# kan-bayashi/espnet

Hardware: AMD Instinct MI355X
Metric: frames/sec, 12L Conformer hybrid CTC/attention training step (B=32 T=1000 d=256 per GPU) (higher is better)
Workload: dtype f32; 1 GPU; BASELINE configs[1]: 12L Conformer enc d=256 h=4 ff=2048 k=31 macaron+cnn rel_pos, 6L Transformer dec, V=5000, fbank B=32 T=1000 L=100, mtlalpha 0.3, lsm 0.1; global_batch=32, frames=1000, parallelism=dp1, optimizer=adam+noam, clip 5.0, launch=hipGraph, wgrad_side_stream=False, optimizer_steps_done=113

## Files before the change

### espnet_amd/csrc/gemm.hip

```cpp
#include <stdlib.h>
#include "common.h"
#include "../../include/espnet_amd.h"

namespace {

constexpr int BK = 32;
constexpr int NTHREADS = 256;

template <int BM, int BN, int PREC>
struct Smem {
  static constexpr int LDK = PREC ? 40 : 36;
  using elem_t = typename std::conditional<PREC == 1, unsigned short, float>::type;
  elem_t a[2][BM][LDK];
  elem_t b[2][BN][LDK];
  int poff[3][BK];
};

struct RowState {
  int base;
  int ih, jw;
  int ok;
};

__device__ __forceinline__ RowState decompose(const eamd_gather_t& g, int row, int nrows) {
// ... 295 lines not shown
          else if (p.epilogue == 3) v = p.aux[coff + prow * p.ldaux + n] > 0.f ? v : 0.f;
          else if (p.epilogue == 4) v *= eamd_dswish(p.aux[coff + prow * p.ldaux + n]);
          else if (p.epilogue == 5) v *= p.aux[coff + prow * p.ldaux + n];
          v *= p.alpha;
          if (p.R) v += p.R[coff + prow * p.ldr + n];
          float* cp = p.C + coff + prow * p.ldc + n;
          if (p.beta != 0.f) v += p.beta * (*cp);
          *cp = v;
        }
      }
    }
  }
}

template <int BM, int BN, int PREC>
int launch(const eamd_gemm_t& p, hipStream_t stream) {
  dim3 grid((p.M + BM - 1) / BM, (p.N + BN - 1) / BN, p.batch1 * p.batch2 * p.splitk);
  size_t smem = sizeof(Smem<BM, BN, PREC>);
  if (smem > 64 * 1024) {
    static const hipError_t attr_err = hipFuncSetAttribute(
        reinterpret_cast<const void*>(&gemm_kernel<BM, BN, PREC>), hipFuncAttributeMaxDynamicSharedMemorySize,
        (int)sizeof(Smem<BM, BN, PREC>));
    if (attr_err != hipSuccess) return (int)attr_err;
  }
  hipLaunchKernelGGL((gemm_kernel<BM, BN, PREC>), grid, dim3(NTHREADS), smem, stream, p);
  EAMD_LAUNCH_CHECK();
  return EAMD_OK;
}

}

int eamd_gemm_bf16_dispatch(const eamd_gemm_t& p, int tile, hipStream_t stream);
int eamd_gemm_f32_dispatch(const eamd_gemm_t& p, int tile, hipStream_t stream);

static int gemm_check(eamd_gemm_t& p, int& tile_out, const bool no_c = false) {
  const bool stats = p.epilogue == 7;
  const bool no_result = stats || no_c;
  const bool rowgrad = p.epilogue == 8;
  if (!p.A || !p.B || (!p.C && !p.Cb && !no_result)) return EAMD_EINVAL;
  if (stats && (!p.stats.part || !p.stats.zfix || (p.stats.col && !p.stats.zcol))) return EAMD_EINVAL;
  if (rowgrad && !p.stats.rowc) return EAMD_EINVAL;
  if ((stats || rowgrad) && (p.stats.fix < 0 || p.stats.fix >= p.N || (p.tile != 64 && p.tile != 128) || p.splitk > 1 ||
                             p.batch1 * p.batch2 != 1 || p.cmap.enabled || p.gather.enabled || p.Hb || p.drop_p != 0.f ||
                             p.R || p.colsum || p.beta != 0.f))
    return EAMD_EINVAL;
  if (p.in_dtype != 0 && p.in_dtype != 1) return EAMD_EINVAL;
  if (p.in_dtype == 1 && p.precision != 1) return EAMD_EINVAL;
  if (p.in_dtype == 0 && (p.Cb || p.aux_dtype || (!p.C && !no_result))) return EAMD_EUNSUPPORTED;
  if (p.M <= 0 || p.N <= 0 || p.K < 0) return EAMD_EINVAL;
  if (p.batch1 <= 0 || p.batch2 <= 0) return EAMD_EINVAL;
  if (p.splitk < 1) p.splitk = 1;
  if (p.splitk > 1 && p.epilogue != 0) return EAMD_EINVAL;
  if (p.epilogue < 0 || p.epilogue > 8) return EAMD_EINVAL;
  if (p.epilogue >= 3 && p.epilogue <= 5 && !p.aux) return EAMD_EINVAL;
  if (p.epilogue == 6 && (!p.Hb || p.drop_p <= 0.f)) return EAMD_EINVAL;
  if (p.precision != 0 && p.precision != 1) return EAMD_EINVAL;
  if ((long)p.batch1 * p.batch2 * p.splitk > 65535) return EAMD_EUNSUPPORTED;

  int tile = p.tile;
  if (tile == 0) {
    long t128 = (long)((p.M + 127) / 128) * ((p.N + 127) / 128) * p.batch1 * p.batch2 * p.splitk;
    if (p.in_dtype == 1) {
      constexpr int T128_KMIN = 320, T128_NMIN = 256;
      tile = (t128 >= 1024 && p.K >= T128_KMIN && p.M >= 2048 && p.N >= T128_NMIN) ? 128 : 64;
    } else {
      tile = (t128 >= (p.precision == 0 ? 240 : 512) && p.M >= 128 && p.N >= 128) ? 128 : 64;
      if (p.precision == 0 && tile == 128 && t128 > 256 && t128 < 400 && p.splitk == 1) tile = 64;
    }
  }
  if (tile != 64 && tile != 128) return EAMD_EINVAL;

  if (p.gather.enabled) {
    const eamd_gather_t& g = p.gather;
    if (g.ntap < 1 || g.ntap > 9 || g.C <= 0 || g.C % BK != 0) return EAMD_EINVAL;
    if (!p.transA) {
      if (p.K != g.ntap * g.C) return EAMD_EINVAL;
    } else {
      if (p.M != g.ntap * g.C) return EAMD_EINVAL;
      if (g.C % tile != 0) return EAMD_EINVAL;
    }
  }
  if (p.colsum && p.gather.enabled &&
      (!p.transA || !p.transB || p.in_dtype != 0 || p.batch1 * p.batch2 != 1 || p.a_act != EAMD_ACT_NONE || p.b_act != EAMD_ACT_NONE))
    return EAMD_EUNSUPPORTED;
  if ((p.N + tile - 1) / tile > 65535) return EAMD_EUNSUPPORTED;
  if (p.h_dtype != 0 && p.h_dtype != 1) return EAMD_EINVAL;
  if (p.in_dtype == 1 && p.h_dtype != 0) return EAMD_EUNSUPPORTED;
  if (p.in_dtype != 1 && ((p.Hb && !(p.h_dtype == 1 && p.precision == 0)) || (p.drop_p != 0.f && p.precision != 0)))
    return EAMD_EUNSUPPORTED;
  if ((p.a_act > EAMD_ACT_SWISH || p.b_act > EAMD_ACT_SWISH) && (p.in_dtype != 0 || p.precision != 0)) return EAMD_EUNSUPPORTED;
  tile_out = tile;
  return EAMD_OK;
}

extern "C" int eamd_gemm(const eamd_gemm_t* pp, void* stream_) {
  if (!pp) return EAMD_EINVAL;
  eamd_gemm_t p = *pp;
  hipStream_t stream = (hipStream_t)stream_;
  int tile = 0;
  const int chk = gemm_check(p, tile);
  if (chk != EAMD_OK) return chk;
  const bool stats = p.epilogue == 7, rowgrad = p.epilogue == 8;
  if (p.in_dtype == 1) return eamd_gemm_bf16_dispatch(p, tile, stream);

  if (p.precision == 1 && p.gather.enabled && p.transA && !p.Hb && p.drop_p == 0.f) {
    const int rc = eamd_gemm_f32_dispatch(p, tile, stream);
    if (rc != EAMD_EUNSUPPORTED) return rc;
  }
  if (p.precision == 0) {
    const int rc = eamd_gemm_f32_dispatch(p, tile, stream);
    if (rc != EAMD_EUNSUPPORTED) return rc;
    if (p.drop_p != 0.f || p.Hb || p.a_act > EAMD_ACT_SWISH || p.b_act > EAMD_ACT_SWISH) return EAMD_EUNSUPPORTED;
  }
  if (stats || rowgrad) return EAMD_EUNSUPPORTED;
  if (p.colsum && p.gather.enabled) return EAMD_EUNSUPPORTED;
  if (tile == 128) {
    return p.precision ? launch<128, 128, 1>(p, stream) : launch<128, 128, 0>(p, stream);
  }
  return p.precision ? launch<64, 64, 1>(p, stream) : launch<64, 64, 0>(p, stream);
}

int eamd_gemm_f32_multi(const eamd_gemm_t* ps, const int* tiles, int n, hipStream_t stream);

extern "C" int eamd_gemm_multi(const eamd_gemm_t* descs, int n, void* stream) {
  if (!descs || n < 1) return EAMD_EINVAL;
  if (n >= 2 && n <= EAMD_GEMM_MULTI_MAX) {
    eamd_gemm_t ps[EAMD_GEMM_MULTI_MAX];
    int tiles[EAMD_GEMM_MULTI_MAX];
    bool f32 = true;
    for (int i = 0; i < n; ++i) {
      ps[i] = descs[i];
      const int chk = gemm_check(ps[i], tiles[i]);
      if (chk != EAMD_OK) return chk;
      f32 = f32 && ps[i].in_dtype == 0 && ps[i].precision == 0;
    }
    if (f32) {
      const int rc = eamd_gemm_f32_multi(ps, tiles, n, (hipStream_t)stream);
      if (rc != EAMD_EUNSUPPORTED) return rc;
    }
  }
  for (int i = 0; i < n; ++i) {
    const int rc = eamd_gemm(&descs[i], stream);
    if (rc != EAMD_OK) return rc;
  }
  return EAMD_OK;
}

int eamd_gemm_f32_conv1w(const eamd_gemm_t* ps, const int* tiles, int n, const float* x, int T, int F, float* part, int* nslab,
                         hipStream_t stream);
int eamd_conv1_bwd_w_reduce(const float* part, int nslab, int C, float* dw, float* db, hipStream_t stream);

extern "C" int eamd_conv2_bwd_x_conv1_bwd_w(const eamd_gemm_t* descs, int n, const float* x, int T, int F, float* part,
// ... 47 lines not shown
```

### espnet_amd/csrc/gemm_f32.hip

```cpp
#include <stdlib.h>
#include <type_traits>
#include "common.h"
#include "../../include/espnet_amd.h"

#include "gemm_bf16_common.h"

namespace {

constexpr int FBK = 32;

template <int BM, int BN, bool TA, bool TB>
struct SmemF {
  static constexpr int KPAD_A = BM >= 128 ? 8 : 4, KPAD_B = BN >= 128 ? 8 : 4;
  static constexpr int LDA = TA ? BM + KPAD_A : FBK + 4;
  static constexpr int RA = TA ? FBK : BM;
  static constexpr int LDB = TB ? BN + KPAD_B : FBK + 4;
  static constexpr int RB = TB ? FBK : BN;
  static constexpr int OPS = 2 * (RA * LDA + RB * LDB);
  static constexpr int CT = BM * (BN + 4);
  float ab[OPS > CT ? OPS : CT];
  int poff[8][FBK];
  __device__ float* a(int buf) { return ab + buf * RA * LDA; }
  __device__ float* b(int buf) { return ab + 2 * RA * LDA + buf * RB * LDB; }
};
// ... 673 lines not shown
}

template <int T>
int dispatch_layout_f(const eamd_gemm_t& p, hipStream_t s) {
  if (p.transA) return p.transB ? launch_f<T, T, true, true, false>(p, s) : launch_f<T, T, true, false, false>(p, s);
  return p.transB ? launch_f<T, T, false, true, false>(p, s) : launch_f<T, T, false, false, false>(p, s);
}

bool aligned16f(const void* q) { return (reinterpret_cast<uintptr_t>(q) & 15) == 0; }

}

int eamd_gemm_f32_dispatch(const eamd_gemm_t& p, int tile, hipStream_t stream) {
  if (p.Cb || (p.Hb && !p.h_dtype) || p.aux_dtype || (!p.C && p.epilogue != 7)) return EAMD_EUNSUPPORTED;
  if (p.Hb && p.drop_p <= 0.f) return EAMD_EINVAL;
  if (p.drop_p < 0.f || p.drop_p >= 1.f) return EAMD_EINVAL;
  if (p.drop_p > 0.f && (p.cmap.enabled || p.batch1 * p.batch2 != 1 || p.ldc != p.N || p.splitk > 1)) return EAMD_EINVAL;
  const bool a_ok = aligned16f(p.A) && p.lda % 4 == 0 && p.sA1 % 4 == 0 && p.sA2 % 4 == 0 &&
                    p.lda >= (p.transA ? (p.M + 3) / 4 * 4 : (p.K + 3) / 4 * 4);
  const bool b_ok = aligned16f(p.B) && p.ldb % 4 == 0 && p.sB1 % 4 == 0 && p.sB2 % 4 == 0 &&
                    p.ldb >= (p.transB ? (p.N + 3) / 4 * 4 : (p.K + 3) / 4 * 4);
  if (p.gather.enabled) {
    const eamd_gather_t& g = p.gather;
    if (g.C % FBK != 0 || !p.transB || !aligned16f(p.A) || !b_ok) return EAMD_EUNSUPPORTED;
    if (p.a_act != EAMD_ACT_NONE || p.b_act != EAMD_ACT_NONE) return EAMD_EUNSUPPORTED;
    if (!gather_taps_small(g)) return EAMD_EUNSUPPORTED;
    if (p.transA && g.C % tile != 0) return EAMD_EUNSUPPORTED;
    if (tile == 128)
      return p.transA ? launch_f<128, 128, true, true, true>(p, stream) : launch_f<128, 128, false, true, true>(p, stream);
    return p.transA ? launch_f<64, 64, true, true, true>(p, stream) : launch_f<64, 64, false, true, true>(p, stream);
  }
  if (!a_ok || !b_ok) return EAMD_EUNSUPPORTED;
  return tile == 128 ? dispatch_layout_f<128>(p, stream) : dispatch_layout_f<64>(p, stream);
}

template <bool NOPAD>
static int multi_launch_t(const MultiF& m, int grid, hipStream_t stream) {
  constexpr size_t smem = sizeof(SmemF<128, 128, false, true>);
  static const hipError_t attr_err = hipFuncSetAttribute(
      reinterpret_cast<const void*>(&gemm_f32_multi_kernel<128, 128, false, true, true, NOPAD>),
      hipFuncAttributeMaxDynamicSharedMemorySize, (int)smem);
  if (attr_err != hipSuccess) return (int)attr_err;
  hipLaunchKernelGGL((gemm_f32_multi_kernel<128, 128, false, true, true, NOPAD>), dim3((unsigned)grid), dim3(NT_), smem, stream, m);
  EAMD_LAUNCH_CHECK();
  return EAMD_OK;
}

int eamd_gemm_f32_multi(const eamd_gemm_t* ps, const int* tiles, int n, hipStream_t stream) {
  if (n < 2 || n > EAMD_GEMM_MULTI_MAX) return EAMD_EUNSUPPORTED;
  MultiF m;
  bool nopad = true;
  int maxnt = 0;
  for (int i = 0; i < n; ++i) {
    const eamd_gemm_t& p = ps[i];
    if (tiles[i] != 128 || p.in_dtype != 0 || p.precision != 0) return EAMD_EUNSUPPORTED;
    if (!p.gather.enabled || p.transA || !p.transB || p.splitk != 1 || p.batch1 * p.batch2 != 1) return EAMD_EUNSUPPORTED;
    if (!p.C || p.Cb || p.Hb || p.aux_dtype || p.epilogue > 5 || p.colsum) return EAMD_EUNSUPPORTED;
    if (p.a_act != EAMD_ACT_NONE || p.b_act != EAMD_ACT_NONE || p.drop_p != 0.f) return EAMD_EUNSUPPORTED;
    const bool b_ok = aligned16f(p.B) && p.ldb % 4 == 0 && p.ldb >= (p.N + 3) / 4 * 4;
    if (p.gather.C % FBK != 0 || !aligned16f(p.A) || !b_ok || !gather_taps_small(p.gather)) return EAMD_EUNSUPPORTED;
    const long nt = (long)((p.M + 127) / 128) * ((p.N + 127) / 128);
    if (nt > (1L << 24)) return EAMD_EUNSUPPORTED;
    nopad = nopad && gather_nopad(p.gather);
    m.p[i] = p;
    m.nt[i] = (int)nt;
    maxnt = nt > maxnt ? (int)nt : maxnt;
// ... 95 lines not shown
```

### espnet_amd/functional.py

```python
import math

import torch

from . import ops
from .ops import (ACT_NONE, ACT_RELU, ACT_SWISH, EPI_DACT_FACTOR, EPI_MUL_AUX, EPI_MUL_DSWISH, EPI_MUL_RELU_MASK, EPI_NONE,
                  EPI_RELU)


class GradSink:

    on_done = None
    on_use = None

    @staticmethod
    def use(params):
        if GradSink.on_use is not None and torch.is_grad_enabled():
            GradSink.on_use(params)
        return params

    def __init__(self, params):
        self.params = list(params)
        self.ret = [None] * len(self.params)

    def buf(self, i):
# ... 584 lines not shown
        adt = ops.act_dtype()
        inp2 = ops.to_act_shared(inp).reshape(-1, Din)
        W = ops.wshadow(ws[0]).detach().as_strided((rows_w, Din), (Din, 1))
        b = bs[0].detach().as_strided((rows_w,), (1,)) if bs else None
        out = ops.linear_fwd(inp2, W, b, out_dtype=adt)
        sp = SharedProj(out, nblk, zero_grad, torch.float32 if zero_grad else adt)
        box.append(sp)
        ctx.sp, ctx.inp2, ctx.W, ctx.shape = sp, inp2, W, inp.shape
        ctx.pr = GradSink.use(params)
        ctx.n_w = n_w
        return torch.zeros((), device=inp.device)

    @staticmethod
    def backward(ctx, _dtoken):
        sp, inp2, W = ctx.sp, ctx.inp2, ctx.W
        params = ctx.pr
        ws, bs = params[:ctx.n_w], params[ctx.n_w:]
        blocks = sorted(sp.pending)
        sp.pending = []
        dinp = None
        if blocks:
            assert blocks == list(range(blocks[0], blocks[-1] + 1)), "consumers of one backward pass are consecutive blocks"
            lo, hi = blocks[0] * sp.width, (blocks[-1] + 1) * sp.width
            M, Din, n = inp2.shape[0], inp2.shape[1], hi - lo
            dy = sp.dout if sp.dout.dtype == inp2.dtype else ops.to_act(sp.dout)
            rows_w = W.shape[0]
            dW = ws[0]._eamd_grad.as_strided((rows_w, Din), (Din, 1))[lo:hi]
            db = bs[0]._eamd_grad.as_strided((rows_w,), (1,))[lo:hi] if bs else None
            sk = ops.auto_splitk(n, Din, M)
            ops.gemm(dy, inp2, dW, n, Din, M, sp.ld, Din, Din, transA=1, transB=1, splitk=sk,
                     beta=1.0 if sk == 1 else 0.0, colsum=db, a_off=lo)
            if ctx.needs_input_grad[0]:
                dinp = torch.empty(M, Din, device=inp2.device, dtype=torch.float32)
                ops.gemm(dy, W, dinp, M, Din, n, sp.ld, Din, Din, transB=1, a_off=lo, b_off=lo * Din)
                dinp = dinp.view(ctx.shape)
            sp.done += len(blocks)
        if sp.done >= sp.n and GradSink.on_done is not None:
            ops.wgrad_join()
            GradSink.on_done(params)
        return (dinp, None, None, None, None) + (None,) * len(params)


class MHABlockFn(torch.autograd.Function):

    @staticmethod
    def forward(ctx, x, memory, pos_emb, mask, H, eps, last_query_only, drop, pre, token, *params):
        p_att, s_att, p_out, s_out = drop
        pre_kv = pre if (pre is not None and pre[0] == "kv") else None
        pre_pos = pre if (pre is not None and pre[0] == "pos") else None
        ln_w, ln_b, wq, bq, wk, bk, wv, bv, wo, bo = params[:10]
        rel = len(params) > 10
        B, T1f, D = x.shape
        dk = D // H
        adt = ops.act_dtype()
        x2 = x.reshape(-1, D).contiguous()
        fused = memory is None and not last_query_only and _qkv_adjacent(wq, wk, wv, bq, bk, bv)
        rp = None
        if fused and eps is not None and D == 256 and x2.dtype == torch.float32 and adt == torch.float32 \
                and ops.rowproj_ok(x2.shape[0], D, 3 * D) and (p_out <= 0.0 or ops.f32_epilogue_drop()):
            w3 = _span3(ops.wshadow(wq), (3 * D, D))
            rp = ops.rowproj_images(wq, [(w3, False), (w3, True), (wo.detach(), False), (wo.detach(), True)])
        if rp is not None:
            xn = torch.empty_like(x2)
            mean = torch.empty(x2.shape[0], device=x2.device, dtype=torch.float32)
            rstd = torch.empty_like(mean)
        else:
            xn, mean, rstd = _ln_fwd_in(x2, ln_w, ln_b, eps, adt)
# ... 638 lines not shown
```

### espnet_amd/ops.py

```python
import ctypes as C
import os
import math

import torch

from . import _lib
from ._lib import GatherT, GemmT, RowMapT, check, ptr, stream_ptr

ACT_NONE, ACT_RELU, ACT_SWISH = 0, 1, 2
EPI_NONE, EPI_RELU, EPI_SWISH, EPI_MUL_RELU_MASK, EPI_MUL_DSWISH, EPI_MUL_AUX, EPI_DACT_FACTOR, EPI_ROW_STATS, EPI_ROW_GRAD = 0, 1, 2, 3, 4, 5, 6, 7, 8

_PRECISIONS = {"fp32": 0, "bf16": 1}
_state = {"precision": 0}


def set_precision(name):
    if name not in _PRECISIONS:
        raise ValueError(f"precision must be one of {list(_PRECISIONS)}")
    _state["precision"] = _PRECISIONS[name]


def get_precision():
    return [k for k, v in _PRECISIONS.items() if v == _state["precision"]][0]

# ... 49 lines not shown


def _span(rows, ld, cols):
    return (rows - 1) * ld + cols if rows > 0 else 0


_time_bound = {"t": None}


def set_time_bound(t):
    if t is not None and not (t.is_cuda and t.dtype == torch.int32 and t.numel() == 1):
        raise _lib.EamdError("time bound: one int32 element on the device")
    _time_bound["t"] = t


def time_bound():
    return _time_bound["t"]


def mask_time(x, T, bound):
    rows = x.numel() // x.shape[-1]
    assert x.is_contiguous() and rows % T == 0 and x.dtype in (torch.float32, torch.bfloat16)
    check(_lib.lib().eamd_mask_time(ptr(x), rows, x.shape[-1], T, ptr(bound), x.dtype == torch.bfloat16,
                                    stream_ptr()), "eamd_mask_time")
    return x


_gemm_record = None


def gemm(A, B, Cm, M, N, K, lda, ldb, ldc, *, transA=0, transB=0, bias=None, aux=None, ldaux=0, R=None,
         ldr=0, batch=(1, 1), sA=(0, 0), sB=(0, 0), sC=(0, 0), alpha=1.0, beta=0.0, a_act=0, b_act=0,
         epilogue=0, splitk=1, tile=0, gather=None, cmap=None, a_off=0, b_off=0, c_off=0, precision=None,
         colsum=None, Cb=None, drop=None, Hb=None, h_act=0, group=False, stats=None, defer=None):
    bf = A.dtype == torch.bfloat16
    if A.dtype != B.dtype or A.dtype not in (torch.float32, torch.bfloat16) or not (A.is_cuda and B.is_cuda):
        raise _lib.EamdError("gemm needs float32 or bfloat16 GPU operands of one dtype")
    if stats is not None:
        assert epilogue in (EPI_ROW_STATS, EPI_ROW_GRAD) and tile in (64, 128) and splitk == 1
        assert (Cm is None and Cb is None) if epilogue == EPI_ROW_STATS else Cm is not None
    c32 = Cm if (Cm is not None and Cm.dtype == torch.float32) else None
    c16 = Cb if Cb is not None else (Cm if (Cm is not None and Cm.dtype == torch.bfloat16) else None)
    if c16 is not None and (c16.dtype != torch.bfloat16 or not bf):
        raise _lib.EamdError("gemm: bf16 outputs need bf16 operands")
    for tt in (R, bias, colsum):
        if tt is not None and tt.dtype != torch.float32:
            raise _lib.EamdError("gemm: bias / residual / colsum must be float32")
    b1, b2 = batch
    if gather is None:
        a_span = _span(K, lda, M) if transA else _span(M, lda, K)
        a_need = a_off + (b1 - 1) * sA[0] + (b2 - 1) * sA[1] + a_span
        if a_need > A.numel():
            raise _lib.EamdError(f"gemm: A too small ({A.numel()} < {a_need})")
    b_span = _span(K, ldb, N) if transB else _span(N, ldb, K)
    b_need = b_off + (b1 - 1) * sB[0] + (b2 - 1) * sB[1] + b_span
    if b_need > B.numel():
        raise _lib.EamdError(f"gemm: B too small ({B.numel()} < {b_need})")
    if cmap is None:
        c_need = c_off + (b1 - 1) * sC[0] + (b2 - 1) * sC[1] + _span(M, ldc, N)
        for ct in (c32, c16):
            if ct is not None and c_need > ct.numel():
                raise _lib.EamdError(f"gemm: C too small ({ct.numel()} < {c_need})")
    if bias is not None and bias.numel() < N:
        raise _lib.EamdError("gemm: bias too small")

    p = GemmT()
    p.A, p.B = ptr(A, a_off), ptr(B, b_off)
# ... 9 lines not shown
                raise _lib.EamdError("gemm: colsum with a gather needs transA, transB, float32 operands and N outputs")
        elif not transA or colsum.numel() < M * b1 * b2:
            raise _lib.EamdError("gemm: colsum needs transA and M outputs")
        p.colsum = ptr(colsum)
    p.M, p.N, p.K = M, N, K
    p.transA, p.transB = int(transA), int(transB)
    p.lda, p.ldb, p.ldc, p.ldaux, p.ldr = lda, ldb, ldc, ldaux or ldc, ldr or ldc
    p.batch1, p.batch2 = b1, b2
    p.sA1, p.sA2 = sA
    p.sB1, p.sB2 = sB
    p.sC1, p.sC2 = sC
    p.alpha, p.beta = alpha, beta
    p.a_act, p.b_act, p.epilogue = a_act, b_act, epilogue
    p.splitk = splitk
    p.in_dtype = 1 if bf else 0
    p.precision = 1 if bf else (_state["precision"] if precision is None else precision)
    p.tile = tile
    if stats is not None and epilogue == EPI_ROW_GRAD:
        rowc, col, fix, gscale, scale = stats
        if rowc.dtype != torch.float32 or rowc.numel() < 3 * M or col.dtype != torch.int32 or col.numel() < M or not (0 <= fix < N):
            raise _lib.EamdError("gemm: row-gradient coefficients too small or of the wrong dtype")
        p.stats.rowc, p.stats.col, p.stats.fix, p.stats.gscale, p.stats.scale = ptr(rowc), ptr(col), int(fix), ptr(gscale), float(scale)
    elif stats is not None:
        part, col, zcol, zfix, fix = stats
        tn = (N + tile - 1) // tile
        if part.dtype != torch.float32 or part.numel() < M * tn * 2 or zfix.numel() < M or not (0 <= fix < N) or \
                (col is not None and (col.dtype != torch.int32 or col.numel() < M or zcol is None or zcol.numel() < M)):
            raise _lib.EamdError("gemm: row-statistics buffers too small or of the wrong dtype")
        p.stats.part, p.stats.col, p.stats.zcol, p.stats.zfix, p.stats.fix = ptr(part), ptr(col), ptr(zcol), ptr(zfix), int(fix)
    if gather is not None:
        p.gather = gather
    if cmap is not None:
        p.cmap = cmap
    if drop is not None and drop[0] > 0.0:
        if ldc != N or c_off != 0 or (not bf and p.precision != 0):
            raise _lib.EamdError("gemm: fused dropout needs a contiguous [M, N] result and bf16 or fp32-MFMA operands")
        p.drop_p, p.drop_salt = float(drop[0]), int(drop[1])
        p.drop_step = ptr(rng_state(A.device))
        if Hb is not None:
            if Hb.dtype != (torch.bfloat16 if bf else torch.float32) or Hb.numel() < M * N:
                raise _lib.EamdError("gemm: Hb must be an [M, N] buffer of the operand dtype")
            p.Hb, p.h_act, p.h_dtype = ptr(Hb), h_act, 0 if bf else 1
    if group and _wgroup["on"] and _in_grad_arena(Cm) and _wgroup_accepts(p):
        lo = Cm.data_ptr() + 4 * c_off
        hi = lo + 4 * _span(M, ldc, N)
        nbytes = A.numel() * A.element_size() + B.numel() * B.element_size()
        clash = any(lo < qhi and qlo < hi and (splitk == 1 or qsk == 1) for qlo, qhi, qsk in _wgroup["ranges"])
        if clash or _wgroup["bytes"] + nbytes > GROUP_WGRAD_MAX_BYTES:
            wgrad_group_flush()
        _wgroup["items"].append((p, (A, B, Cm, colsum)))
        _wgroup["ranges"].append((lo, hi, splitk))
        _wgroup["bytes"] += nbytes
        return
    if defer is not None:
        defer.append((p, (A, B, Cm, bias, aux, R, colsum, Cb, Hb, stats)))
        return
    if _gemm_record is not None:
        _gemm_record.append((p, (A, B, Cm, bias, aux, R, colsum, Cb, Hb, stats),
                             lambda sp, p=p: check(_lib.lib().eamd_gemm(C.byref(p), sp), "eamd_gemm")))
    check(_lib.lib().eamd_gemm(C.byref(p), stream_ptr()), "eamd_gemm")


GEMM_MULTI_MAX = 4


def gemm_multi(items):
# ... 187 lines not shown
        with inference():
            return fn(*a, **k)
    return wrapped
LINEAR_ROWS_MAX = 16
LINEAR_ROWS_BLOCK_MAX = 1024
LINEAR_ROWS_KSPLIT = True


def linear_fwd(x, W, b, out=None, *, act=EPI_NONE, R=None, alpha=1.0, a_act=ACT_NONE, out_dtype=torch.float32,
               drop=None, Hb=None, h_act=ACT_NONE):
    M, K = x.shape
    N = W.shape[0]
    assert W.shape[1] == K and W.is_contiguous() and x.stride(1) == 1 and (R is None or R.stride(-1) == 1)
    if (LINEAR_ROWS and (M <= LINEAR_ROWS_MAX or (M <= LINEAR_ROWS_BLOCK_MAX and (K <= 512 or (K >= 1024 and LINEAR_ROWS_KSPLIT)) and N <= 1024
                                                  and K % 16 == 0)) and out is None and out_dtype == torch.float32 and x.dtype == torch.float32 and W.dtype == torch.float32
            and act in (EPI_NONE, EPI_RELU, EPI_SWISH) and a_act in (ACT_NONE, ACT_RELU, ACT_SWISH) and drop is None and Hb is None
            and K % 4 == 0 and _state["precision"] == 0 and _infer > 0 and not torch.is_grad_enabled()
            and (R is None or (tuple(R.shape) == (M, N) and (M == 1 or R.stride(0) >= N))) and (M == 1 or x.stride(0) >= K)):
        y = torch.empty(M, N, device=x.device, dtype=torch.float32)
        rc = _lib.lib().eamd_linear_rows_f32(ptr(x), ptr(W), ptr(b), ptr(R), ptr(y), M, N, K, a_act, act, alpha,
                                             x.stride(0), R.stride(0) if R is not None else 0, stream_ptr())
        if rc == 0:
            return y
        if rc != _lib.EAMD_EUNSUPPORTED:
            check(rc, "eamd_linear_rows_f32")
    x = x.contiguous()
    R = R.contiguous() if R is not None else None
    sk = 1
    if (out_dtype if out is None else out.dtype) == torch.float32 and act == EPI_NONE and drop is None and Hb is None:
        if R is None and alpha == 1.0:
            sk = _skinny_splitk(M, N, K)
        elif K >= 1024 and M <= 512 and x.is_cuda and torch.cuda.is_current_stream_capturing():
            sk = _skinny_splitk(M, N, K, max_rows=512)
    if out is None:
        out = zeros(M, N, device=x.device) if sk > 1 else torch.empty(M, N, device=x.device, dtype=out_dtype)
    elif sk > 1:
        out.zero_()
    gemm(x, W, out, M, N, K, K, K, N, bias=b, epilogue=act, R=R, ldr=N, alpha=alpha, a_act=a_act, drop=drop, Hb=Hb,
         h_act=h_act, splitk=sk)
    return out


class _ZeroArena:
    buf = None
    off = 0
    need = 0
    cap = 0
    active = False
    tracking = False
    capture = 0


_zarena = _ZeroArena()
ZERO_ARENA = True
ZERO_ARENA_MAX = 1024 << 20


def _capture_id():
    if not torch.cuda.is_available() or not torch.cuda.is_current_stream_capturing():
        return 0
    try:
        from . import graphs
        return graphs.capture_id()
    except Exception:
        return -1

# ... 20 lines not shown
    for d in shape:
        n *= int(d)
    a = _zarena
    nb = (n * 4 + 255) // 256 * 256
    if a.tracking:
        a.need += nb
    if a.active and n > 0 and a.off + nb <= a.buf.numel() * 4 and a.buf.device == torch.device(device) \
            and (not a.buf.is_cuda or _capture_id() == a.capture):
        t = a.buf[a.off // 4: a.off // 4 + n].view(shape)
        a.off += nb
        return t
    return torch.zeros(shape, device=device, dtype=torch.float32)


def _skinny_splitk(M, N, K, max_rows=64):
    if M > max_rows or N * K < 512 * 512:
        return 1
    tiles = (M + 63) // 64 * ((N + 63) // 64)
    sk = 1
    while tiles * sk < 256 and K // (sk * 2) >= 128:
        sk *= 2
    return sk


def linear_bwd_x(dy, W, out=None, *, beta=0.0, epilogue=EPI_NONE, aux=None, alpha=1.0, out_dtype=torch.float32,
                 drop=None):
    M, N = dy.shape
    K = W.shape[1]
    assert W.shape[0] == N and dy.is_contiguous()
    fresh = out is None
    sk = 1
    if fresh and out_dtype == torch.float32 and epilogue == EPI_NONE and aux is None and drop is None and alpha == 1.0:
        sk = _skinny_splitk(M, K, N)
    if out is None:
        assert beta == 0.0
        out = zeros(M, K, device=dy.device) if sk > 1 else torch.empty(M, K, device=dy.device, dtype=out_dtype)
    gemm(dy, W, out, M, K, N, N, K, K, transB=1, beta=beta, epilogue=epilogue, aux=aux, ldaux=K, alpha=alpha,
         drop=drop, splitk=sk)
    return out


FUSED_FFN = True
FUSED_FFN_MIN_ROWS = 4096


def ffn_fused_ok(x, w1, w2, act):
    bf = x.dtype == torch.bfloat16
    if not FUSED_FFN or x.dtype != w1.dtype or w1.dtype != w2.dtype or (bf and _state["precision"] != 1) or \
            (not bf and (x.dtype != torch.float32 or _state["precision"] != 0)):
        return False
    return (x.shape[1] == 256 and w1.shape[1] == 256 and w1.shape[0] % (256 if bf else 128) == 0 and w1.shape[0] >= 256
            and tuple(w2.shape) == (256, w1.shape[0]) and act in (ACT_RELU, ACT_SWISH)
            and (x.shape[0] >= FUSED_FFN_MIN_ROWS or ffn_hsplit(x.shape[0], w1.shape[0], bf) > 1))


FUSED_FFN_HSPLIT_MIN_ROWS = 1536


def ffn_hsplit(M, F, bf):
    if bf or M >= FUSED_FFN_MIN_ROWS or M < FUSED_FFN_HSPLIT_MIN_ROWS or F % 256 != 0 or F < 512:
        return 1
    return 2


def _ffn_desc(x, w1, b1, w2, b2, R, out, f, h, act, alpha, drop, F=None):
    p = _lib.FfnT()
# ... 216 lines not shown


def enable_wgrad_stream(enable=True):
    _wgrad["stream"] = torch.cuda.Stream() if enable else None
    _wgrad["used"] = False


def wgrad_group_end():
    wgrad_group_flush()
    _wgroup["on"] = False


def wgrad_join():
    wgrad_group_flush()
    st = _wgrad["stream"]
    if st is not None and _wgrad["used"]:
        torch.cuda.current_stream().wait_stream(st)
        _wgrad["used"] = False


def linear_bwd_w(dy, x, dW, *, alpha=1.0, b_act=ACT_NONE, db=None, group=True):
    st = _wgrad["stream"]
    if st is None:
        return _linear_bwd_w(dy, x, dW, alpha=alpha, b_act=b_act, db=db, group=group)
    cur = torch.cuda.current_stream()
    st.wait_stream(cur)
    with torch.cuda.stream(st):
        _linear_bwd_w(dy, x, dW, alpha=alpha, b_act=b_act, db=db)
    dy.record_stream(st)
    x.record_stream(st)
    _wgrad["used"] = True


def _linear_bwd_w(dy, x, dW, *, alpha=1.0, b_act=ACT_NONE, db=None, group=True):
    M, N = dy.shape
    K = x.shape[1]
    assert x.shape[0] == M and dW.numel() == N * K and dW.dtype == torch.float32
    grouping = group and _wgroup["on"] and _wgrad["stream"] is None
    if (grouping and M <= STACK_WGRAD_MAX_ROWS and alpha == 1.0 and b_act == ACT_NONE
            and dy.is_contiguous() and x.is_contiguous() and _in_grad_arena(dW)):
        key = (dW.data_ptr(), db.data_ptr() if db is not None else 0, dy.dtype, x.dtype, N, K)
        _wgroup["stack"].setdefault(key, (dW, db, [], []))
        ent = _wgroup["stack"][key]
        ent[2].append(dy)
        ent[3].append(x)
        return
    sk = auto_splitk(N, K, M)
    tile = 0
    t64 = ((N + 63) // 64) * ((K + 63) // 64)
    if grouping and t64 <= GROUP_WGRAD_MAX_TILES and _in_grad_arena(dW):
        if t64 >= GROUP_WGRAD_TILE128_MIN and N >= 128 and K >= 128 and dy.dtype == torch.float32 and _state["precision"] == 0:
            tile = 128
            sk = max(1, min(GROUP_WGRAD_T128_WGS // (((N + 127) // 128) * ((K + 127) // 128)), M // 256))
        else:
            tile = 64
            sk = max(1, sk // GROUP_WGRAD_SK_DIV)
    gemm(dy, x, dW, N, K, M, N, K, K, transA=1, transB=1, alpha=alpha, b_act=b_act, splitk=sk, tile=tile,
         beta=1.0 if sk == 1 else 0.0, colsum=db, group=grouping)


def colsum(x, out, scale=1.0, rows=None, D=None, ld=None):
    rows = x.shape[0] if rows is None else rows
    D = x.shape[1] if D is None else D
    ld = D if ld is None else ld
    assert out.numel() >= D
    check(_lib.lib().eamd_colsum(ptr(x), ld, ptr(out), rows, D, scale,
                                 1 if x.dtype == torch.bfloat16 else 0, stream_ptr()), "eamd_colsum")


def layernorm_fwd(x, gamma, beta, eps, out_dtype=torch.float32):
    rows, D = x.shape
    y = torch.empty(rows, D, device=x.device, dtype=out_dtype)
    mean = torch.empty(rows, device=x.device, dtype=torch.float32)
    rstd = torch.empty(rows, device=x.device, dtype=torch.float32)
    y32, y16 = (ptr(y), None) if out_dtype == torch.float32 else (None, ptr(y))
    check(_lib.lib().eamd_layernorm_fwd(ptr(x), ptr(gamma), ptr(beta), y32, y16, ptr(mean), ptr(rstd), rows, D,
                                        eps, stream_ptr()), "eamd_layernorm_fwd")
    return y, mean, rstd


class _LnReduceJob(C.Structure):
    _fields_ = [("ws", C.c_void_p), ("dgamma", C.c_void_p), ("dbeta", C.c_void_p), ("nblk", C.c_int32), ("D", C.c_int32)]


defer_ln_reduce = True
_ln_pending = []
_ln_task = -1


# ... 2294 lines not shown
```

### include/espnet_amd.h

```cpp
#ifndef ESPNET_AMD_H_
#define ESPNET_AMD_H_
#include <stdint.h>
#ifdef __cplusplus
extern "C" {
#endif

int eamd_abi_version(void);

typedef struct {
  int32_t enabled;
  int32_t C;
  int32_t ntap;
  int32_t Ho, Wo;
  int32_t Hin, Win;
  int32_t sh, sw;
  int32_t dh[9], dw[9];
} eamd_gather_t;

typedef struct {
  int32_t enabled;
  int32_t Ho, Wo;
  int32_t Hc, Wc;
  int32_t sh, oh, sw, ow;
} eamd_rowmap_t;

typedef struct {
  const float* A; const float* B; float* C;
  const float* bias; const float* aux; const float* R;
  float* colsum;
  int32_t M, N, K;
  int32_t transA, transB;
  int64_t lda, ldb, ldc, ldaux, ldr;
  int32_t batch1, batch2;
  int64_t sA1, sA2, sB1, sB2, sC1, sC2;
  float alpha, beta;
  int32_t a_act, b_act, epilogue;
  int32_t splitk;
  int32_t precision;
  int32_t tile;
  eamd_gather_t gather;
  eamd_rowmap_t cmap;
  void* Cb;
  int32_t in_dtype;
  int32_t aux_dtype;
  float drop_p;
  uint64_t drop_salt;
  const uint64_t* drop_step;
  void* Hb;
  int32_t h_act;
  int32_t h_dtype;
  struct {
    float* part; const int32_t* col; float* zcol; float* zfix; int32_t fix; int32_t reserved;
    const float* rowc; const float* gscale; float scale; int32_t reserved2;
  } stats;
} eamd_gemm_t;

int eamd_gemm(const eamd_gemm_t* p, void* stream);

#define EAMD_GEMM_MULTI_MAX 4
int eamd_gemm_multi(const eamd_gemm_t* descs, int n, void* stream);

int eamd_conv2_bwd_x_conv1_bwd_w(const eamd_gemm_t* descs, int n, const float* x, int T, int F, float* part, float* dw,
                                 float* db, void* stream);

int eamd_gemm_group_plan(const eamd_gemm_t* descs, int n, int32_t* first);
int eamd_gemm_group_launch(const eamd_gemm_t* descs_dev, const int32_t* first_dev, int n, int total, int in_dtype, int tile,
                           void* stream);

typedef struct {
  const float* x; const float* w1; const float* b1; const float* w2; const float* b2; const float* R;
  float* out; float* f; float* h;
  int32_t M, D, F, act;
  float alpha;
  float p_in; uint64_t salt_in; float p_out; uint64_t salt_out; const void* drop_step;
  int32_t dtype;
  int32_t hsplit;
  const float* ln_x; const float* ln_w; const float* ln_b; float* ln_mean; float* ln_rstd;
  float ln_eps; int32_t reserved2;
  const float* lnb_x; const float* lnb_gamma; const float* lnb_mean; const float* lnb_rstd; const float* lnb_dres;
  float* lnb_ws; float* lnb_drop_out; uint64_t lnb_drop_salt; float lnb_drop_p; int32_t reserved3;
} eamd_ffn_t;
int eamd_ffn_fwd(const eamd_ffn_t* p, void* stream);
int eamd_ffn_bwd(const eamd_ffn_t* p, void* stream);
typedef struct {
  const float* w1; const float* w2;
  float* fwd_first; float* fwd_second; float* bwd_first; float* bwd_second;
  int32_t D, F;
} eamd_ffn_pack_t;
int eamd_ffn_pack_f32_multi(const eamd_ffn_pack_t* jobs, int njobs, void* stream);

// ... 468 lines not shown
```

Baseline: 1.140 million frames/s.

## Add occupancy-aware split-K and tile planner for large fp32 GEMMs

Adds a host-side planner that looks up the per-CU resident workgroup count through the occupancy API. For large fp32 GEMMs it picks a tile size and split-K factor that reduce the empty tail wave. The Python callers now pass splitk=0 to opt in for forward, dgrad and wgrad GEMMs. When the split is above one and beta is 0, the output buffer is zeroed asynchronously first. The aim is better CU utilisation on GEMMs whose tile count fills the last wave poorly, at the cost of an extra memset, atomic or partial accumulation traffic, and more host-side dispatch logic.

```diff
diff --git a/espnet_amd/csrc/gemm.hip b/espnet_amd/csrc/gemm.hip
--- a/espnet_amd/csrc/gemm.hip
+++ b/espnet_amd/csrc/gemm.hip
@@ -351,8 +351,69 @@
 
 int eamd_gemm_bf16_dispatch(const eamd_gemm_t& p, int tile, hipStream_t stream);
 int eamd_gemm_f32_dispatch(const eamd_gemm_t& p, int tile, hipStream_t stream);
-
-static int gemm_check(eamd_gemm_t& p, int& tile_out, const bool no_c = false) {
+int eamd_gemm_f32_resident(const eamd_gemm_t& p, int tile);
+
+
+static int fp32_default_tile(int M, int N, long t128, int precision, int splitk) {
+  int tile = (t128 >= (precision == 0 ? 240 : 512) && M >= 128 && N >= 128) ? 128 : 64;
+  if (precision == 0 && tile == 128 && t128 > 256 && t128 < 400 && splitk == 1) tile = 64;
+  return tile;
+}
+
+static long plan_tiles(int M, int N, int tile) { return (long)((M + tile - 1) / tile) * ((N + tile - 1) / tile); }
+static double plan_cost(long W, long R) { return (double)((W + R - 1) / R) * (double)R / (double)W; }
+static double plan_last_empty(long W, long R) { return (double)(((W + R - 1) / R) * R - W) / (double)R; }
+
+static int plan_split_for(long tiles, long R, int smax) {
+  if (plan_last_empty(tiles, R) < 0.10) return 1;
+  int best = 1;
+  double best_cost = plan_cost(tiles, R);
+  for (int s = 2; s <= smax; ++s) {
+    const double c = plan_cost(tiles * s, R);
+    if (c < best_cost - 1e-9) { best = s; best_cost = c; }
+  }
+  return best;
+}
+
+static bool plan_big(int M, int N, int K, int wgrad) {
+  constexpr int ROWS_MIN = 4096;
+  return wgrad ? K >= ROWS_MIN : (M >= ROWS_MIN || (M >= ROWS_MIN / 2 && (N >= ROWS_MIN || K >= ROWS_MIN)));
+}
+
+extern "C" int eamd_gemm_split_plan(int M, int N, int K, int wgrad, int accumulate, int r64, int r128, int32_t* tile_out,
+                                    int32_t* split_out) {
+  if (M <= 0 || N <= 0 || K < 0 || !tile_out || !split_out) return EAMD_EINVAL;
+  constexpr int MIN_KTILES = 16;
+  const long t128 = plan_tiles(M, N, 128);
+  if (!plan_big(M, N, K, wgrad) || r64 <= 0 || r128 <= 0) {
+    *tile_out = fp32_default_tile(M, N, t128, 0, 1);
+    *split_out = 1;
+    return EAMD_OK;
+  }
+  const int nkt = (K + BK - 1) / BK;
+  int smax = nkt / MIN_KTILES;
+  smax = smax < 1 ? 1 : smax > 64 ? 64 : smax;
+  if (!accumulate && smax > 2) smax = 2;
+  int tile = fp32_default_tile(M, N, wgrad ? t128 * smax : t128, 0, wgrad ? smax : 1);
+  int s = plan_split_for(plan_tiles(M, N, tile), tile == 128 ? r128 : r64, smax);
+  if (tile == 128 && plan_last_empty(t128 * s, r128) > 0.25) {
+    const long t64 = plan_tiles(M, N, 64);
+    const int s64 = plan_split_for(t64, r64, smax);
+    if (plan_last_empty(t64 * s64, r64) <= 0.25) { tile = 64; s = s64; }
+  }
+  *tile_out = tile;
+  *split_out = s;
+  return EAMD_OK;
+}
+
+static bool plan_eligible(const eamd_gemm_t& p) {
+  if (p.in_dtype != 0 || p.precision != 0 || p.epilogue != 0 || p.drop_p != 0.f || p.Hb || p.Cb || !p.C) return false;
+  if (p.gather.enabled || p.cmap.enabled || p.batch1 * p.batch2 != 1 || p.tile != 0) return false;
+  if (p.beta == 1.f) return true;
+  return p.beta == 0.f && p.ldc == p.N && p.R != p.C;
+}
+
+static int gemm_check(eamd_gemm_t& p, int& tile_out, const bool no_c = false, bool* planned = nullptr) {
   const bool stats = p.epilogue == 7;
   const bool no_result = stats || no_c;
   const bool rowgrad = p.epilogue == 8;
@@ -368,6 +429,16 @@
   if (p.in_dtype == 0 && (p.Cb || p.aux_dtype || (!p.C && !no_result))) return EAMD_EUNSUPPORTED;
   if (p.M <= 0 || p.N <= 0 || p.K < 0) return EAMD_EINVAL;
   if (p.batch1 <= 0 || p.batch2 <= 0) return EAMD_EINVAL;
+  int plan_tile = 0;
+  if (p.splitk == 0 && planned && plan_eligible(p) && plan_big(p.M, p.N, p.K, p.transA && p.transB)) {
+    const int r64 = eamd_gemm_f32_resident(p, 64), r128 = eamd_gemm_f32_resident(p, 128);
+    int32_t pt = 0, ps = 1;
+    const int rc = eamd_gemm_split_plan(p.M, p.N, p.K, p.transA && p.transB, p.beta == 1.f, r64, r128, &pt, &ps);
+    if (rc != EAMD_OK) return rc;
+    plan_tile = pt;
+    p.splitk = ps;
+    *planned = ps > 1;
+  }
   if (p.splitk < 1) p.splitk = 1;
   if (p.splitk > 1 && p.epilogue != 0) return EAMD_EINVAL;
   if (p.epilogue < 0 || p.epilogue > 8) return EAMD_EINVAL;
@@ -376,15 +447,14 @@
   if (p.precision != 0 && p.precision != 1) return EAMD_EINVAL;
   if ((long)p.batch1 * p.batch2 * p.splitk > 65535) return EAMD_EUNSUPPORTED;
 
-  int tile = p.tile;
+  int tile = plan_tile ? plan_tile : p.tile;
   if (tile == 0) {
     long t128 = (long)((p.M + 127) / 128) * ((p.N + 127) / 128) * p.batch1 * p.batch2 * p.splitk;
     if (p.in_dtype == 1) {
       constexpr int T128_KMIN = 320, T128_NMIN = 256;
       tile = (t128 >= 1024 && p.K >= T128_KMIN && p.M >= 2048 && p.N >= T128_NMIN) ? 128 : 64;
     } else {
-      tile = (t128 >= (p.precision == 0 ? 240 : 512) && p.M >= 128 && p.N >= 128) ? 128 : 64;
-      if (p.precision == 0 && tile == 128 && t128 > 256 && t128 < 400 && p.splitk == 1) tile = 64;
+      tile = fp32_default_tile(p.M, p.N, t128, p.precision, p.splitk);
     }
   }
   if (tile != 64 && tile != 128) return EAMD_EINVAL;
@@ -417,8 +487,13 @@
   eamd_gemm_t p = *pp;
   hipStream_t stream = (hipStream_t)stream_;
   int tile = 0;
-  const int chk = gemm_check(p, tile);
+  bool planned = false;
+  const int chk = gemm_check(p, tile, false, &planned);
   if (chk != EAMD_OK) return chk;
+  if (planned && p.beta == 0.f) {
+    const int zrc = eamd_zero_async(p.C, (size_t)p.M * p.N * sizeof(float), stream);
+    if (zrc != EAMD_OK) return zrc;
+  }
   const bool stats = p.epilogue == 7, rowgrad = p.epilogue == 8;
   if (p.in_dtype == 1) return eamd_gemm_bf16_dispatch(p, tile, stream);
 
@@ -437,6 +512,18 @@
     return p.precision ? launch<128, 128, 1>(p, stream) : launch<128, 128, 0>(p, stream);
   }
   return p.precision ? launch<64, 64, 1>(p, stream) : launch<64, 64, 0>(p, stream);
+}
+
+extern "C" int eamd_gemm_plan(const eamd_gemm_t* pp, int32_t* tile, int32_t* split) {
+  if (!pp || !tile || !split) return EAMD_EINVAL;
+  eamd_gemm_t p = *pp;
+  int t = 0;
+  bool planned = false;
+  const int chk = gemm_check(p, t, false, &planned);
+  if (chk != EAMD_OK) return chk;
+  *tile = t;
+  *split = p.splitk;
+  return EAMD_OK;
 }
 
 int eamd_gemm_f32_multi(const eamd_gemm_t* ps, const int* tiles, int n, hipStream_t stream);
diff --git a/espnet_amd/csrc/gemm_f32.hip b/espnet_amd/csrc/gemm_f32.hip
--- a/espnet_amd/csrc/gemm_f32.hip
+++ b/espnet_amd/csrc/gemm_f32.hip
@@ -729,6 +729,48 @@
   }
   if (!a_ok || !b_ok) return EAMD_EUNSUPPORTED;
   return tile == 128 ? dispatch_layout_f<128>(p, stream) : dispatch_layout_f<64>(p, stream);
+}
+
+namespace {
+
+template <int BM, int BN, bool TA, bool TB, int ACT>
+int resident_f2() {
+  static const int r = [] {
+    constexpr size_t smem = sizeof(SmemF<BM, BN, TA, TB>);
+    const void* fn = reinterpret_cast<const void*>(&gemm_f32_kernel<BM, BN, TA, TB, false, ACT, false, false>);
+    int dev = 0, cus = 0, per_cu = 0;
+    if (smem > 64 * 1024 && hipFuncSetAttribute(fn, hipFuncAttributeMaxDynamicSharedMemorySize, (int)smem) != hipSuccess) return 0;
+    if (hipGetDevice(&dev) != hipSuccess) return 0;
+    if (hipDeviceGetAttribute(&cus, hipDeviceAttributeMultiprocessorCount, dev) != hipSuccess) return 0;
+    if (hipOccupancyMaxActiveBlocksPerMultiprocessor(&per_cu, fn, NT_, smem) != hipSuccess) return 0;
+    return per_cu > 0 && cus > 0 ? per_cu * cus : 0;
+  }();
+  return r;
+}
+
+template <int T, bool TA, bool TB>
+int resident_f(const eamd_gemm_t& p) {
+  if (p.a_act > EAMD_ACT_SWISH || p.b_act > EAMD_ACT_SWISH) return resident_f2<T, T, TA, TB, 2>();
+  if (p.a_act != EAMD_ACT_NONE || p.b_act != EAMD_ACT_NONE) return resident_f2<T, T, TA, TB, 1>();
+  return resident_f2<T, T, TA, TB, 0>();
+}
+
+template <int T>
+int resident_layout_f(const eamd_gemm_t& p) {
+  if (p.transA) return p.transB ? resident_f<T, true, true>(p) : resident_f<T, true, false>(p);
+  return p.transB ? resident_f<T, false, true>(p) : resident_f<T, false, false>(p);
+}
+
+}
+
+int eamd_gemm_f32_resident(const eamd_gemm_t& p, int tile) {
+  if (p.in_dtype != 0 || p.precision != 0 || p.gather.enabled || p.epilogue >= 7 || !p.C || p.Cb || p.Hb || p.aux_dtype) return 0;
+  const bool a_ok = aligned16f(p.A) && p.lda % 4 == 0 && p.sA1 % 4 == 0 && p.sA2 % 4 == 0 &&
+                    p.lda >= (p.transA ? (p.M + 3) / 4 * 4 : (p.K + 3) / 4 * 4);
+  const bool b_ok = aligned16f(p.B) && p.ldb % 4 == 0 && p.sB1 % 4 == 0 && p.sB2 % 4 == 0 &&
+                    p.ldb >= (p.transB ? (p.N + 3) / 4 * 4 : (p.K + 3) / 4 * 4);
+  if (!a_ok || !b_ok) return 0;
+  return tile == 128 ? resident_layout_f<128>(p) : resident_layout_f<64>(p);
 }
 
 template <bool NOPAD>
diff --git a/espnet_amd/functional.py b/espnet_amd/functional.py
--- a/espnet_amd/functional.py
+++ b/espnet_amd/functional.py
@@ -640,7 +640,8 @@
                      beta=1.0 if sk == 1 else 0.0, colsum=db, a_off=lo)
             if ctx.needs_input_grad[0]:
                 dinp = torch.empty(M, Din, device=inp2.device, dtype=torch.float32)
-                ops.gemm(dy, W, dinp, M, Din, n, sp.ld, Din, Din, transB=1, a_off=lo, b_off=lo * Din)
+                ops.gemm(dy, W, dinp, M, Din, n, sp.ld, Din, Din, transB=1, a_off=lo, b_off=lo * Din,
+                         splitk=0 if dy.dtype == torch.float32 else 1)
                 dinp = dinp.view(ctx.shape)
             sp.done += len(blocks)
         if sp.done >= sp.n and GradSink.on_done is not None:
diff --git a/espnet_amd/ops.py b/espnet_amd/ops.py
--- a/espnet_amd/ops.py
+++ b/espnet_amd/ops.py
@@ -105,7 +105,7 @@
 def gemm(A, B, Cm, M, N, K, lda, ldb, ldc, *, transA=0, transB=0, bias=None, aux=None, ldaux=0, R=None,
          ldr=0, batch=(1, 1), sA=(0, 0), sB=(0, 0), sC=(0, 0), alpha=1.0, beta=0.0, a_act=0, b_act=0,
          epilogue=0, splitk=1, tile=0, gather=None, cmap=None, a_off=0, b_off=0, c_off=0, precision=None,
-         colsum=None, Cb=None, drop=None, Hb=None, h_act=0, group=False, stats=None, defer=None):
+         colsum=None, Cb=None, drop=None, Hb=None, h_act=0, group=False, stats=None, defer=None, plan=False):
     bf = A.dtype == torch.bfloat16
     if A.dtype != B.dtype or A.dtype not in (torch.float32, torch.bfloat16) or not (A.is_cuda and B.is_cuda):
         raise _lib.EamdError("gemm needs float32 or bfloat16 GPU operands of one dtype")
@@ -181,6 +181,10 @@
         p.gather = gather
     if cmap is not None:
         p.cmap = cmap
+    if plan:
+        pt, ps = C.c_int32(0), C.c_int32(0)
+        check(_lib.lib().eamd_gemm_plan(C.byref(p), C.byref(pt), C.byref(ps)), "eamd_gemm_plan")
+        return pt.value, ps.value
     if drop is not None and drop[0] > 0.0:
         if ldc != N or c_off != 0 or (not bf and p.precision != 0):
             raise _lib.EamdError("gemm: fused dropout needs a contiguous [M, N] result and bf16 or fp32-MFMA operands")
@@ -434,6 +438,8 @@
             sk = _skinny_splitk(M, N, K)
         elif K >= 1024 and M <= 512 and x.is_cuda and torch.cuda.is_current_stream_capturing():
             sk = _skinny_splitk(M, N, K, max_rows=512)
+        if sk == 1 and x.dtype == torch.float32:
+            sk = 0
     if out is None:
         out = zeros(M, N, device=x.device) if sk > 1 else torch.empty(M, N, device=x.device, dtype=out_dtype)
     elif sk > 1:
@@ -520,6 +526,9 @@
     sk = 1
     if fresh and out_dtype == torch.float32 and epilogue == EPI_NONE and aux is None and drop is None and alpha == 1.0:
         sk = _skinny_splitk(M, K, N)
+    if sk == 1 and fresh and out_dtype == torch.float32 and dy.dtype == torch.float32 and epilogue == EPI_NONE and aux is None \
+            and drop is None:
+        sk = 0
     if out is None:
         assert beta == 0.0
         out = zeros(M, K, device=dy.device) if sk > 1 else torch.empty(M, K, device=dy.device, dtype=out_dtype)
@@ -802,6 +811,9 @@
     _wgrad["used"] = True
 
 
+PLAN_MIN_ROWS = 4096
+
+
 def _linear_bwd_w(dy, x, dW, *, alpha=1.0, b_act=ACT_NONE, db=None, group=True):
     M, N = dy.shape
     K = x.shape[1]
@@ -825,6 +837,9 @@
         else:
             tile = 64
             sk = max(1, sk // GROUP_WGRAD_SK_DIV)
+    if tile == 0 and dy.dtype == torch.float32 and _state["precision"] == 0 and M >= PLAN_MIN_ROWS:
+        gemm(dy, x, dW, N, K, M, N, K, K, transA=1, transB=1, alpha=alpha, b_act=b_act, splitk=0, beta=1.0, colsum=db)
+        return
     gemm(dy, x, dW, N, K, M, N, K, K, transA=1, transB=1, alpha=alpha, b_act=b_act, splitk=sk, tile=tile,
          beta=1.0 if sk == 1 else 0.0, colsum=db, group=grouping)
 
diff --git a/include/espnet_amd.h b/include/espnet_amd.h
--- a/include/espnet_amd.h
+++ b/include/espnet_amd.h
@@ -56,6 +56,10 @@
 } eamd_gemm_t;
 
 int eamd_gemm(const eamd_gemm_t* p, void* stream);
+
+int eamd_gemm_plan(const eamd_gemm_t* p, int32_t* tile, int32_t* split);
+
+int eamd_gemm_split_plan(int M, int N, int K, int wgrad, int accumulate, int r64, int r128, int32_t* tile, int32_t* split);
 
 #define EAMD_GEMM_MULTI_MAX 4
 int eamd_gemm_multi(const eamd_gemm_t* descs, int n, void* stream);
```

Measured after the change: 1.143 million frames/s (median of 6 runs). No clear change (+0.3%).
